# traveller59/spconv

Measured on AMD Instinct MI355X. Metric: active-voxels/sec fwd+bwd, 3x3x3 SubMConv3d C=64, ~100k voxels/scene, higher is better.
Workload: dtype f16; 1 GPU; SubMConv3d 3x3x3 C=64->64 f16, 100000 uniform voxels/scene in 1600x1280x40 (BASELINE configs[1]), 8 distinct scenes per GPU visited round-robin, rulebook reused via indice_key; voxels_per_gpu=100000, launch=hipgraph, steps_per_replay=8, scenes_rotated=8, mask_sort=False, prewarm_steps=0, parallelism=dp1, ranks_seen=1, tree=unknown

## Files before the change

include/spconv_amd.h:

```cpp
#ifndef SPCONV_AMD_H_
#define SPCONV_AMD_H_

#include <stddef.h>
#include <stdint.h>

#ifdef __cplusplus
extern "C" {
#endif

#define SPX_MAX_NDIM 4
#define SPX_UNION_MAX_OPERANDS 8
#define SPX_COLLAPSE_SUM 0
#define SPX_COLLAPSE_MEAN 1
#define SPX_COLLAPSE_MAX 2
#define SPX_SCORE_ABSMEAN 0
#define SPX_SCORE_ABSMAX 1

typedef void *spx_stream_t;

enum spx_dtype { SPX_F32 = 0, SPX_F16 = 1, SPX_BF16 = 2, SPX_I8 = 3, SPX_F64 = 4 };

enum spx_act { SPX_ACT_NONE = 0, SPX_ACT_RELU = 1, SPX_ACT_SIGMOID = 2, SPX_ACT_LEAKY_RELU = 3 };
#define SPX_OUT_CACHED 0x100
#define SPX_TILE_ORDER 0x200

const char *spx_last_error(void);

int spx_version(void);

int spx_set_option(const char *name_h, int value);

long long spx_launch_count(const char *family_h);

int spx_pad_rows(const void *src, void *dst, long long rows, int src_row_bytes, int dst_row_bytes,
                 spx_stream_t stream);

int spx_conv_out_shape(int ndim, const int *in_shape, const int *ksize, const int *stride,
                       const int *padding, const int *dilation, const int *out_padding,
                       int transposed, int *out_shape);


size_t spx_subm_rulebook_ws_bytes(int n, int kv);

int spx_subm_rulebook(const int32_t *indices, int n, int ndim, int batch_size,
                      const int *spatial_shape, const int *ksize, const int *dilation,
                      int32_t *pair_fwd, int32_t *pair_bwd, uint32_t *mask,
                      int32_t *pair_native, int32_t *num_per_loc,
                      void *ws, size_t ws_bytes, spx_stream_t stream);

size_t spx_conv_rulebook_ws_bytes(int n_in, int ndim, const int *ksize, const int *stride,
                                  const int *dilation, int transposed);

int spx_conv_rulebook_count(const int32_t *indices, int n_in, int ndim, int batch_size,
                            const int *in_shape, const int *out_shape, const int *ksize,
                            const int *stride, const int *padding, const int *dilation,
// ... 394 lines not shown
```

spconv_amd/_lib.py:

```python
from __future__ import annotations

import ctypes
import os
import subprocess
from typing import Optional

_HERE = os.path.dirname(os.path.abspath(__file__))
LIB_PATH = os.environ.get("SPX_LIB") or os.path.join(_HERE, "lib", "libspconv_amd.so")

c_int_p = ctypes.POINTER(ctypes.c_int)
c_float_p = ctypes.POINTER(ctypes.c_float)
vp = ctypes.c_void_p

SIGNATURES = {
    "spx_last_error": (ctypes.c_char_p, []),
    "spx_version": (ctypes.c_int, []),
    "spx_set_option": (ctypes.c_int, [ctypes.c_char_p, ctypes.c_int]),
    "spx_conv_out_shape": (ctypes.c_int, [ctypes.c_int] + [c_int_p] * 6 + [ctypes.c_int, c_int_p]),
    "spx_subm_rulebook_ws_bytes": (ctypes.c_size_t, [ctypes.c_int, ctypes.c_int]),
    "spx_subm_rulebook": (ctypes.c_int, [vp, ctypes.c_int, ctypes.c_int, ctypes.c_int, c_int_p,
                                         c_int_p, c_int_p, vp, vp, vp, vp, vp, vp,
                                         ctypes.c_size_t, vp]),
    "spx_conv_rulebook_ws_bytes": (ctypes.c_size_t, [ctypes.c_int, ctypes.c_int, c_int_p, c_int_p,
                                                     c_int_p, ctypes.c_int]),
# ... 84 lines not shown
                                       vp, vp, vp, vp, c_int_p, vp, ctypes.c_size_t, vp]),
    "spx_point2voxel_static_ws_bytes": (ctypes.c_size_t, [ctypes.c_int] * 4 + [c_int_p, ctypes.c_int]),
    "spx_point2voxel_static": (ctypes.c_int, [vp, vp, ctypes.c_int, vp, ctypes.c_int, ctypes.c_int,
                                              ctypes.POINTER(ctypes.c_float), ctypes.POINTER(ctypes.c_float), c_int_p]
                               + [ctypes.c_int] * 5 + [vp] * 6 + [ctypes.c_int, vp, ctypes.c_size_t, vp,
                                                                  ctypes.c_size_t, vp]),
    "spx_hash_ws_bytes": (ctypes.c_size_t, [ctypes.c_int]),
    "spx_hash_clear": (ctypes.c_int, [vp, ctypes.c_int, ctypes.c_int, vp]),
    "spx_hash_insert": (ctypes.c_int, [vp, vp, ctypes.c_int, ctypes.c_int, ctypes.c_int, vp, vp, ctypes.c_int, vp]),
    "spx_hash_query": (ctypes.c_int, [vp, vp, ctypes.c_int, ctypes.c_int, ctypes.c_int, vp, vp, vp, ctypes.c_int, vp]),
    "spx_hash_insert_exist": (ctypes.c_int, [vp, vp, ctypes.c_int, ctypes.c_int, ctypes.c_int, vp, vp, vp,
                                             ctypes.c_int, vp]),
    "spx_hash_assign_arange": (ctypes.c_int, [vp, vp, ctypes.c_int, ctypes.c_int, ctypes.c_int, vp, vp,
                                              ctypes.c_size_t, vp]),
    "spx_hash_items": (ctypes.c_int, [vp, vp, ctypes.c_int, ctypes.c_int, ctypes.c_int, vp, vp, ctypes.c_int, vp,
                                      vp, ctypes.c_size_t, vp]),
    "spx_rankmap_from_sorted": (ctypes.c_int, [vp, ctypes.c_int, ctypes.c_int, ctypes.c_int, c_int_p, vp,
                                               ctypes.c_size_t, vp, vp]),
    "spx_key_argsort_ws_bytes": (ctypes.c_size_t, [ctypes.c_int]),
    "spx_key_argsort": (ctypes.c_int, [vp, ctypes.c_int, ctypes.c_int, ctypes.c_int, c_int_p, vp, vp, vp,
                                       ctypes.c_size_t, vp, vp, vp, ctypes.c_int, vp, ctypes.c_size_t, vp]),
    "spx_pad_rows": (ctypes.c_int, [vp, vp, ctypes.c_longlong, ctypes.c_int, ctypes.c_int, vp]),
    "spx_launch_count": (ctypes.c_longlong, [ctypes.c_char_p]),
    "spx_bias_act_inplace": (ctypes.c_int, [vp, vp, ctypes.c_int, ctypes.c_int, ctypes.c_int,
                                            ctypes.c_int, ctypes.c_float, vp]),
    "spx_dense_ws_bytes": (ctypes.c_size_t, [ctypes.c_int, ctypes.c_int, c_int_p]),
    "spx_dense_map": (ctypes.c_int, [vp, ctypes.c_int, vp, ctypes.c_int, ctypes.c_int, c_int_p, vp, vp]),
    "spx_to_dense": (ctypes.c_int, [vp, ctypes.c_int, ctypes.c_longlong, vp, vp, ctypes.c_int, ctypes.c_int, ctypes.c_int,
                                    ctypes.c_longlong, ctypes.c_int, ctypes.c_int, c_int_p, vp]),
    "spx_dense_gather": (ctypes.c_int, [vp, vp, vp] + [ctypes.c_int] * 6 + [c_int_p, vp]),
    "spx_from_dense_ws_bytes": (ctypes.c_size_t, [ctypes.c_int, ctypes.c_int, c_int_p]),
    "spx_from_dense_count": (ctypes.c_int, [vp] + [ctypes.c_int] * 5 + [c_int_p, vp, ctypes.c_size_t, c_int_p, vp]),
    "spx_from_dense_fill": (ctypes.c_int, [vp] + [ctypes.c_int] * 4 + [c_int_p, vp, ctypes.c_size_t, vp, vp, vp, vp]),
    "spx_union_ws_bytes": (ctypes.c_size_t, [ctypes.c_int, ctypes.c_int, c_int_p, ctypes.c_int, ctypes.c_longlong]),
    "spx_union_count": (ctypes.c_int, [vp, c_int_p, vp, ctypes.c_int, ctypes.c_int, ctypes.c_int, c_int_p, vp,
                                       ctypes.c_size_t, vp, ctypes.c_size_t, c_int_p, vp]),
    "spx_union_fill": (ctypes.c_int, [vp, c_int_p, vp, ctypes.c_int, ctypes.c_int, ctypes.c_int, c_int_p, ctypes.c_int,
                                      ctypes.c_int, vp, vp, vp, vp, ctypes.c_size_t, vp, ctypes.c_size_t, vp]),
    "spx_union_static": (ctypes.c_int, [vp, c_int_p, vp, ctypes.c_int, ctypes.c_int, ctypes.c_int, c_int_p, ctypes.c_int,
                                        vp, vp, vp, vp, vp, ctypes.c_size_t, vp, ctypes.c_size_t, vp]),
    "spx_union_add_fwd": (ctypes.c_int, [vp, c_int_p, ctypes.c_int, vp, ctypes.c_int, ctypes.c_int, ctypes.c_int, vp, vp,
                                         vp]),
    "spx_union_add_bwd": (ctypes.c_int, [vp, ctypes.c_int, vp, vp, c_int_p, ctypes.c_int, ctypes.c_int, ctypes.c_int,
                                         vp]),
    "spx_collapse_ws_bytes": (ctypes.c_size_t, [ctypes.c_int, ctypes.c_int, c_int_p, ctypes.c_int, ctypes.c_longlong]),
    "spx_collapse_count": (ctypes.c_int, [vp, ctypes.c_int, vp, ctypes.c_int, ctypes.c_int, c_int_p, ctypes.c_int, vp,
# ... 134 lines not shown
```

spconv_amd/csrc/counters.cpp:

```cpp
#include "counters.h"

#include <string.h>

#include "../../include/spconv_amd.h"

namespace spx {
std::atomic<long long> g_counters[kCounterSlots];

namespace {
#define SPX_COUNTER_NAME(e, key) key,
const char *const kNames[] = {SPX_COUNTERS(SPX_COUNTER_NAME)};
#undef SPX_COUNTER_NAME
static_assert(sizeof(kNames) / sizeof(kNames[0]) == kNamed, "one name per enumerator");

template <int N>
int index_of(const char *t, const char *const (&names)[N]) {
  for (int i = 0; i < N; ++i)
    if (strcmp(t, names[i]) == 0) return i;
  return -1;
}

int parse_dt(const char *t) {
  static const char *const names[inst::kDts] = {"f16", "bf16", "i8", "f32"};
  return index_of(t, names);
}

int parse_int(const char *t) {
  if (!*t || strlen(t) > 6) return -1;
  int v = 0;
  for (; *t; ++t) {
// ... 66 lines not shown
  if (named >= 0) return named;
  char buf[96];
  if (strlen(key) >= sizeof(buf)) return -1;
  strcpy(buf, key);
  const char *tok[8];
  int n = 0;
  for (char *c = buf, *start = buf;; ++c) {
    if (*c == '/' || *c == 0) {
      if (n == 8) return -1;
      const bool end = *c == 0;
      *c = 0;
      tok[n++] = start;
      start = c + 1;
      if (end) break;
    }
  }
  const int i = instance_slot(tok, n);
  if (i >= 0) return kInstBase + i;
  const int p = pool_key_slot(tok, n);
  return p < 0 ? -1 : kPoolBase + p;
}
}

extern "C" long long spx_launch_count(const char *family_h) {
  const int slot = family_h ? spx::counter_slot(family_h) : -1;
  return slot < 0 ? -1 : spx::g_counters[slot].load(std::memory_order_relaxed);
}
```

spconv_amd/csrc/counters.h:

```cpp
#pragma once
#include <atomic>

namespace spx {

#define SPX_COUNTERS(X)                                                                                               \
  X(kFamV4, "igemm_v4") X(kFamWs, "igemm_ws") X(kFamBwdFused, "igemm_bwd") X(kFamBwdRows, "igemm_bwd_rows")           \
  X(kFamI8Stream, "igemm_i8_stream") X(kFamGeneric, "generic") X(kFamStage2, "wgrad_stage2")                          \
  X(kFamStage2Batch, "wgrad_stage2_batch") X(kFamF64, "igemm_f64") X(kFamV4w, "igemm_v4w")                            \
  X(kHintV4, "sparse_hint/v4") X(kHintBwd, "sparse_hint/bwd")                                                         \
  X(kF64Fwd, "igemm_f64/fwd") X(kF64Dgrad, "igemm_f64/dgrad") X(kF64Wgrad, "wgrad_f64") X(kF64Pool, "pool/f64")       \
  X(kDenseMap, "dense/map") X(kDenseScatterCl, "dense/scatter_cl") X(kDenseScatterCf, "dense/scatter_cf")             \
  X(kDenseGatherCl, "dense/gather_cl") X(kDenseGatherCf, "dense/gather_cf") X(kDenseCompact, "dense/compact")         \
  X(kUnionMark, "union/mark") X(kUnionPrefix, "union/prefix") X(kUnionClaim, "union/claim")                           \
  X(kUnionFill, "union/fill") X(kUnionAddFwd, "union/add_fwd") X(kUnionAddBwd, "union/add_bwd")                       \
  X(kCollapseMark, "collapse/mark") X(kCollapsePrefix, "collapse/prefix") X(kCollapseRank, "collapse/rank")           \
  X(kCollapseList, "collapse/list") X(kCollapseFwd, "collapse/fwd") X(kCollapseBwd, "collapse/bwd")                   \
  X(kPvGroups, "pointvoxel/groups") X(kPvGather, "pointvoxel/gather") X(kPvDecorate, "pointvoxel/decorate")           \
  X(kInterpCornersRanked, "interp/corners_ranked") X(kInterpCornersHash, "interp/corners_hash")                       \
  X(kInterpFwd, "interp/fwd") X(kInterpBwd, "interp/bwd")                                                             \
  X(kQueryRanked, "query/ranked") X(kQueryHash, "query/hash") X(kQueryGroupFwd, "query/group_fwd")                    \
  X(kQueryGroupBwd, "query/group_bwd")                                                                                \
  X(kSampleFps, "sample/fps") X(kSampleBallQuery, "sample/ball_query") X(kSampleKnnQuery, "sample/knn_query")         \
  X(kBoxCorners, "box/corners") X(kBoxPairs, "box/pairs") X(kBoxAligned, "box/aligned") X(kBoxKey, "box/key")         \
  X(kBoxMask, "box/mask") X(kBoxReduce, "box/reduce")                                                                 \
// ... 58 lines not shown
}
constexpr int v4w(int dt, bool bt, int nks, int pk) {
  return kV4w + ((dt * 2 + (bt ? 1 : 0)) * 2 + (nks - 1)) * kWidePks + pk_slot(pk);
}
}

enum PoolDt { kPoolF16 = 0, kPoolBf16, kPoolF32, kPoolF64, kPoolI8, kPoolDts };
constexpr int kPoolOps = 4, kPoolCount = kPoolOps * kPoolDts * 2;
constexpr int pool_slot(int op, int dt, bool scalar) { return (op * kPoolDts + dt) * 2 + (scalar ? 1 : 0); }

constexpr int kInstBase = kNamed, kPoolBase = kInstBase + inst::kCount, kCounterSlots = kPoolBase + kPoolCount;
extern std::atomic<long long> g_counters[kCounterSlots];

inline void count(Counter c) { g_counters[c].fetch_add(1, std::memory_order_relaxed); }
template <int I>
inline void count_inst() {
  static_assert(I >= 0 && I < inst::kCount, "instance counter slot");
  g_counters[kInstBase + I].fetch_add(1, std::memory_order_relaxed);
}
inline void count_pool(int op, int dt, bool scalar) {
  g_counters[kPoolBase + pool_slot(op, dt, scalar)].fetch_add(1, std::memory_order_relaxed);
}

const char *counter_name(int c);
int counter_slot(const char *key);

}
```

spconv_amd/csrc/igemm_bwd.h:

```cpp
#pragma once
#include "igemm_v4.h"

namespace spx {
namespace {

constexpr int kWT = 64;

constexpr int kW2MaxG = 1024;
constexpr int kW2J = 128;
constexpr int kW2Rec = 8;
constexpr int kXcds = 8;


__host__ __device__ inline int plan2_wg(int w) { return 8 + kW2Rec * w; }
__host__ __device__ inline int plan2_kf(int G) { return 8 + kW2Rec * G; }
__host__ __device__ inline int plan2_seg(int G, int kv) { return 8 + kW2Rec * G + kv + 1; }
__host__ __device__ inline int plan2_red(int G, int kv) {
  return (plan2_seg(G, kv) + 3 * (G + kv) + 3) & ~3;
}

__device__ __forceinline__ int wtr_x(int row) { return ((row >> 1) & 1) | (((row >> 3) & 1) << 1); }
__device__ __forceinline__ int wtr_slot(int row, int sl) {
  return row * 128 + ((((sl >> 1) ^ wtr_x(row)) << 5) | ((sl & 1) << 4));
}
// ... 289 lines not shown
int launch_bwd(const GemmParams &p, const Wgrad2Params &q, int n_wgrad_blocks, hipStream_t s) {
  int napp = p.cls ? layout_app_tiles(p.n_dst, 64 * MB) : 0;
  AppShape exact{-1, 0};
  if constexpr (DT == 0 || DT == 1) {
    if (p.cls) exact = app_shape_exact(p.n_dst, 64 * MB, p.app_m, kAppBudget);
  }
  if (exact.napp >= 0) napp = exact.napp;
  const int n_dgrad = div_up(p.n_dst, 64 * MB) + napp;
  GemmRest rr = rest_of(p);
  rr.napp = p.cls ? napp : -1;
  if (exact.napp >= 0) {
    rr.acc_mode = pack_app_shape(p.acc_mode, p.app_m, exact);
    count(kHintBwd);
  }
  constexpr int wgrad_first = 1;
  GemmParams pl = p;
  pl.lpt = p.tile_order && n_dgrad + n_wgrad_blocks > 1024;
  count(kFamBwdFused);
#define SPX_LAUNCH_BWD(NKSV, PKV)                                                                                  \
  do {                                                                                                               \
    count_inst<inst::bwd(COUT, MB, DT, NKSV, PKV)>();                                                                \
    hipLaunchKernelGGL((igemm_bwd_kernel<COUT, MB, DT, NKSV, PKV>), dim3(n_dgrad + n_wgrad_blocks), dim3(kThreads),  \
                       (bwd_smem_bytes<COUT, MB, DT>()), s, p.A, p.B, p.mask, p.argsort, p.pair, p.n_dst,           \
                       p.n_src, p.CIN, p.kv, p.identity_k, v4_flags(pl), rr,                                        \
                       wgrad_first ? ~n_wgrad_blocks : n_dgrad, q);                                                 \
  } while (0)
  const int pk = v4_pack(p, DT, DT == 3 ? 4 : 2, true);
  if constexpr (DT == 0 || DT == 1) {
    if (pk == 32) SPX_LAUNCH_BWD(2, 32);
    else if (pk == 16) SPX_LAUNCH_BWD(2, 16);
    else if (pk == 8) SPX_LAUNCH_BWD(2, 8);
    else if (pk == 4) SPX_LAUNCH_BWD(1, 4);
    else if (pk == 2) SPX_LAUNCH_BWD(1, 2);
    else if (p.CIN * 2 <= 64) SPX_LAUNCH_BWD(1, 1);
    else SPX_LAUNCH_BWD(2, 1);
  } else {
    if (p.CIN * (DT == 3 ? 4 : 2) <= 64) SPX_LAUNCH_BWD(1, 1);
    else SPX_LAUNCH_BWD(2, 1);
  }
#undef SPX_LAUNCH_BWD
  SPX_LAUNCH_CHECK();
  return 0;
}

template <int DT>
int dispatch_bwd(const GemmParams &p, const Wgrad2Params &q, int nwb, hipStream_t s) {
  switch (p.COUT) {
    case 16: return launch_bwd<16, 2, DT>(p, q, nwb, s);
    case 32: return launch_bwd<32, 2, DT>(p, q, nwb, s);
    case 64: return launch_bwd<64, 2, DT>(p, q, nwb, s);
// ... 8 lines not shown
```

spconv_amd/csrc/igemm_defs.h:

```cpp
#pragma once
#include "common.h"

#include <stdlib.h>
#include <type_traits>
#include <utility>

#ifndef SPX_AUX_TABLE
#define SPX_AUX_TABLE 0
#endif
#ifndef SPX_WD
#define SPX_WD 2
#endif
#ifndef SPX_AUX_OUT
#define SPX_AUX_OUT 2
#endif

namespace spx {

struct GemmParams {
  const void *A;
  const void *B;
  void *out;
  const int32_t *pair;
  const uint32_t *mask;
// ... 6 lines not shown
  int tile_order;
  int kbase, mask_words;
  float *acc;
  int acc_mode;
  int act;
  float act_alpha;
  const float *scale;
  const void *add;
  float add_scale;
  int out_dtype;
  int dbg;
  int xcd_rot;
  int lpt;
  const int32_t *cls;
  const uint32_t *mask_rows;
  int app_rows;
  int app_budget;
  int app_m;
  int app_h;
  int dense_hint;
  float *stats;
  const int32_t *n_live;
  int *grid_out;
  int n0;
};

constexpr int kAppBudget = 64;
constexpr int kLayoutMinRows = 32768;
__host__ __device__ inline int layout_mcap(int n) { return ((n / 4 + 63) & ~63) + 256; }
__host__ __device__ inline int layout_app_tiles(int n, int tm) { return (n / 4 + tm - 1) / tm; }

inline void apply_rows_layout(GemmParams &p, int tile_order) {
  p.cls = nullptr;
  p.mask_rows = nullptr;
  p.app_rows = 0;
  p.app_budget = 0;
  p.app_m = -1;
  p.app_h = 0;
  if (tile_order == SPX_ROWS_LAYOUT && p.argsort && p.pair && p.mask) {
    const int32_t *blob = p.argsort;
    const size_t npad = (static_cast<size_t>(p.n_dst) + 63) & ~static_cast<size_t>(63);
    p.cls = blob;
    p.mask_rows = p.mask;
    p.mask = reinterpret_cast<const uint32_t *>(blob + SPX_LAYOUT_HEADER);
    p.argsort = blob + SPX_LAYOUT_HEADER + npad;
    p.tile_order = 0;
// ... 410 lines not shown
```

spconv_amd/csrc/igemm_v4.h:

```cpp
#pragma once
#include "igemm_defs.h"

namespace spx {
namespace {

#ifdef SPX_TIMELINE
constexpr int kTlSlots = 8, kTlMaxWg = 8192;
__device__ unsigned long long g_timeline[kTlMaxWg * kTlSlots];
#define SPX_STAMP(i)                                                                     \
  do {                                                                                   \
    if (threadIdx.x == 0 && blockIdx.x < kTlMaxWg)                                       \
      g_timeline[blockIdx.x * kTlSlots + (i)] = __builtin_amdgcn_s_memtime();            \
  } while (0)
#else
#define SPX_STAMP(i) do {} while (0)
#endif




template <int COUT, int MB, int DT, bool BT, int NKS = 2, int PK = 1, bool WIDE = false>
__device__ __forceinline__ void igemm_v4_body(const GemmParams &p, int block);
__device__ __forceinline__ void unpack_gemm_args(GemmParams &p, const void *argA, const void *argB,
                                                 const uint32_t *arg_mask, const int32_t *arg_argsort,
                                                 const int32_t *arg_pair, int n_dst, int n_src, int CIN,
                                                 int kv, int identity_k, int b_reverse,
                                                 const GemmRest &rest);

template <int COUT, int MB, int DT, bool BT, int NKS = 2, int PK = 1>
__global__ void __launch_bounds__(kThreads)
igemm_v4_kernel(const void *argA, const void *argB, const uint32_t *arg_mask,
                const int32_t *arg_argsort, const int32_t *arg_pair, int n_dst, int n_src, int CIN,
                int kv, int identity_k, int b_reverse, GemmRest rest) {
  GemmParams p;
  unpack_gemm_args(p, argA, argB, arg_mask, arg_argsort, arg_pair, n_dst, n_src, CIN, kv, identity_k,
                   b_reverse, rest);
  igemm_v4_body<COUT, MB, DT, BT, NKS, PK>(p, blockIdx.x);
}

__device__ __forceinline__ void unpack_gemm_args(GemmParams &p, const void *argA, const void *argB,
                                                 const uint32_t *arg_mask, const int32_t *arg_argsort,
                                                 const int32_t *arg_pair, int n_dst, int n_src, int CIN,
                                                 int kv, int identity_k, int b_reverse,
                                                 const GemmRest &rest) {
  p.A = argA;
  p.B = argB;
  p.mask = arg_mask;
  p.argsort = arg_argsort;
  p.pair = arg_pair;
  p.n_dst = n_dst;
  p.n_src = n_src;
  p.CIN = CIN;
  p.kv = kv;
  p.identity_k = identity_k;
  p.b_reverse = b_reverse & 1;
  p.tile_order = (b_reverse >> 1) & 1;
  p.mask_words = ((b_reverse >> 2) & 3) + 1;
  p.kbase = (b_reverse >> 4) & 127;
  p.lpt = (b_reverse >> 11) & 1;
  p.acc = rest.acc;
  p.acc_mode = rest.acc_mode & 3;
  p.out = rest.out;
  p.bias = rest.bias;
  p.strideK = rest.strideK;
  p.strideN = rest.strideN;
  p.strideD = rest.strideD;
  p.COUT = rest.COUT;
  p.act = rest.act;
  p.act_alpha = rest.act_alpha;
  p.scale = rest.scale;
  p.add = rest.add;
  p.add_scale = rest.add_scale;
  p.out_dtype = rest.out_dtype;
  p.dbg = rest.dbg;
  p.xcd_rot = 0;
  p.stats = rest.stats;
  p.n_live = rest.n_live;
  p.app_rows = rest.napp;
  p.app_budget = 0;
  p.app_m = ((rest.acc_mode >> 8) & 0xfffff) - 1;
  p.app_h = ((rest.acc_mode >> 4) & 15) * 16;
  p.cls = nullptr;
// ... 61 lines not shown
        addw[mb][nb] = word;
      } else if (p.out_dtype == SPX_F32) {
        uint32_t d[4];
#pragma unroll
        for (int e = 0; e < 4; ++e) d[e] = __builtin_bit_cast(uint32_t, v[e]);
        store_dwords<4, SPX_AUX_OUT>(d, rO, rowoff[mb] == kOob ? kOob : (rowoff[mb] + nb * 4) * 4u);
      } else {
        uint32_t d[2];
#pragma unroll
        for (int q = 0; q < 2; ++q)
          d[q] = p.out_dtype == SPX_BF16 ? pack2<true>(v[2 * q], v[2 * q + 1])
                                         : pack2<false>(v[2 * q], v[2 * q + 1]);
        store_dwords<2, SPX_AUX_OUT>(d, rO, rowoff[mb] == kOob ? kOob : (rowoff[mb] + nb * 4) * 2u);
      }
    }
  }
  if (p.out_dtype == SPX_I8) {
#pragma unroll
    for (int mb = 0; mb < MB; ++mb) store_dwords<CPL / 4, SPX_AUX_OUT>(addw[mb], rO, rowoff[mb]);
  }

}

template <int COUT, int MB, int DT, bool BT, int NKS, int PK, bool WIDE>
__device__ __forceinline__ void igemm_v4_body(const GemmParams &p, int block) {
  constexpr bool BF16 = DT == 1, I8 = DT == 2, F32 = DT == 3;
  constexpr bool XK = PK >= 8;
  constexpr int PP = XK ? PK / 8 : PK;
  constexpr int T = PP * (XK ? 2 : 1);
  static_assert(PK == 1 || (!I8 && !F32 && (XK ? NKS == 2 : NKS == 1)), "offset packing: 16-bit operands");
  static_assert(PP == 1 || PP == 2 || PP == 4, "offsets per piece");
  constexpr int ES = I8 ? 1 : (F32 ? 4 : 2);
  static_assert(!(I8 && BT), "int8 is forward only");
  constexpr int NB = COUT / 16;
  const int ldo = WIDE ? p.COUT : COUT;
  const int n0 = WIDE ? p.n0 : 0;
  constexpr int TM = 64 * MB;
  constexpr int BROWS = !BT ? (COUT + 31) / 32 : (F32 ? (COUT + 31) / 32 : 2 * ((COUT + 63) / 64));
  constexpr int BA = BROWS < 2 ? 2 : BROWS;
  constexpr int B_BYTES = COUT * kRowBytes;
  constexpr int CPL = NB * 4;
  extern __shared__ __attribute__((aligned(16))) char smem[];
  uint32_t *lds_mask = reinterpret_cast<uint32_t *>(smem + 2 * B_BYTES);
  float *lds_sb = reinterpret_cast<float *>(smem + 2 * B_BYTES + 64);

  SPX_STAMP(0);
  const int tid = threadIdx.x, lane = tid & 63, wave = tid >> 6;
  const int ntiles = (p.n_dst + TM - 1) / TM;
  const int napp = p.cls ? (p.app_rows >= 0 ? p.app_rows : layout_app_tiles(p.n_dst, TM)) : 0;
  const bool app = block < napp;
  int app_m = 0;
  int tile = 0;
  int pos[MB];
  if (app) {
    app_m = p.app_m;
    int h = p.app_h;
    if (app_m < 0) {
      typedef const i32x2 __attribute__((address_space(4))) *cptr_t;
      const i32x2 head = *(cptr_t)(p.cls);
      const int cls = head[0];
      app_m = head[1];
      if (!cls) {
        if constexpr (!I8 && !BT && !WIDE) if (p.stats) wg_bn_stats_empty<COUT>(p.stats, block, static_cast<int>(gridDim.x));
        return;
// ... 11 lines not shown
      const int q = block * h + blk * 16 + (threadIdx.x & 15);
      pos[mb] = (blk * 16 < h && q < app_m) ? q : -1;
    }
    tile = block;
  } else {
    const int bid = block - napp;
    const int rot = (p.xcd_rot + napp) & 7;
    tile = (p.tile_order && p.lpt) ? ntiles - 1 - bid : (rot ? xcd_tile_rot(bid, ntiles, rot) : xcd_tile(bid, ntiles));
#pragma unroll
    for (int mb = 0; mb < MB; ++mb) {
      const int t = tile * TM + ((threadIdx.x >> 6) * MB + mb) * 16 + (threadIdx.x & 15);
      pos[mb] = t < p.n_dst ? t : -1;
    }
  }
  const int mcap = layout_mcap(p.n_dst);
  const int32_t *order_app = p.argsort;
  const uint32_t *maskp = app ? reinterpret_cast<const uint32_t *>(order_app + mcap) : p.mask;
  const int32_t *pairp = app ? order_app + 2 * static_cast<size_t>(mcap) : p.pair;
  const int tbl_rows = app ? mcap : p.n_dst;
  const int lrow = lane & 15, lgrp = lane >> 4;
  const int slot = tid & 7, r0 = tid >> 3;
  constexpr int GL = 4 / PP;
  const int ga = lgrp / GL;
  auto swzB = [](int row, int sl) __attribute__((always_inline)) {
    const int x = ((row >> 1) & 1) | (((row / CPL) & 3) << 1);
    return row * kRowBytes + ((sl ^ x) << 4);
  };
  const uint32_t rowB = static_cast<uint32_t>(p.CIN) * ES;
  const int nchunk = (static_cast<int>(rowB) + kRowBytes - 1) / kRowBytes;
  const bool cfull = (rowB & (kRowBytes - 1)) == 0;

  const uint32_t a_bytes = static_cast<uint32_t>(p.n_src) * rowB;
  const uint32_t w_bytes = static_cast<uint32_t>(p.COUT) * p.kv * rowB;
  const uint32_t pair_bytes = static_cast<uint32_t>(tbl_rows) * 4u;

  const int32_t *olist = (app || !p.cls) ? p.argsort : nullptr;
  const bool by_row = olist && !app && !p.tile_order;
  const __amdgpu_buffer_rsrc_t rO = make_rsrc(olist, olist ? pair_bytes : 0u);
  int glist[MB];
  uint32_t goff[MB];
#pragma unroll
  for (int mb = 0; mb < MB; ++mb) {
    goff[mb] = pos[mb] < 0 ? kOob : static_cast<uint32_t>(pos[mb]) * 4u;
    glist[mb] = static_cast<int>(__builtin_amdgcn_raw_buffer_load_b32(rO, goff[mb], 0, SPX_AUX_TABLE));
  }
  if (by_row) {
#pragma unroll
    for (int mb = 0; mb < MB; ++mb) goff[mb] = pos[mb] < 0 ? kOob : static_cast<uint32_t>(glist[mb]) * 4u;
    asm volatile("" ::: "memory");
  }
// ... 287 lines not shown
    if (!SPX_ABL(p, 1) && !SPX_ABL(p, 2)) store_b(smem + (1 - S) * B_BYTES, WSetN{});
    compute(it0, SET);
    const StepIt it3 = step_next<T>(it2, nchunk);
    if (!SPX_ABL(p, 1) && !SPX_ABL(p, 2)) {
      if constexpr (WD == 2) load_b(it3, WSetN{});
      else load_b(it2, WSetN{});
    }
    __builtin_amdgcn_sched_barrier(0);
    load_idx(it3, std::integral_constant<int, 1 - S>{});
    __builtin_amdgcn_sched_barrier(0);
    load_a(it2, SET);
    it0 = it1;
    it1 = it2;
    it2 = it3;
  };
  SPX_STAMP(3);
  while (it0.k >= 0) {
    step(Set1{});
    step(Set0{});
  }
  SPX_STAMP(4);

  if constexpr (!I8) {
    const bool plain = p.bias == nullptr && p.act == SPX_ACT_NONE;
    const __amdgpu_buffer_rsrc_t rO = make_rsrc(p.out, static_cast<uint32_t>(p.n_dst) * (ldo * ES));
    float bv[CPL];
#pragma unroll
    for (int q = 0; q < CPL; ++q) bv[q] = 0.f;
    if (p.bias) {
#pragma unroll
      for (int q = 0; q < CPL; ++q) {
        if constexpr (F32) bv[q] = static_cast<const float *>(p.bias)[n0 + lgrp * CPL + q];
        else bv[q] = to_float<BF16>(static_cast<const uint16_t *>(p.bias)[n0 + lgrp * CPL + q]);
      }
    }
    if (p.acc_mode) {
      const __amdgpu_buffer_rsrc_t rS = make_rsrc(p.acc, static_cast<uint32_t>(p.n_dst) * (ldo * 4));
#pragma unroll
      for (int mb = 0; mb < MB; ++mb) {
        const uint32_t so = grow[mb] < 0 ? kOob : static_cast<uint32_t>(grow[mb]) * (ldo * 4) + (n0 + lgrp * CPL) * 4;
        uint32_t prev[CPL];
        if (p.acc_mode & 1) load_dwords<CPL>(prev, rS, so);
#pragma unroll
        for (int nb = 0; nb < NB; ++nb)
#pragma unroll
          for (int e = 0; e < 4; ++e) {
            if (p.acc_mode & 1) acc[nb][mb][e] += __builtin_bit_cast(float, prev[nb * 4 + e]);
            prev[nb * 4 + e] = __builtin_bit_cast(uint32_t, static_cast<float>(acc[nb][mb][e]));
          }
        if (p.acc_mode & 2) store_dwords<CPL>(prev, rS, so);
      }
      if (p.acc_mode & 2) return;
    }
#pragma unroll
    for (int mb = 0; mb < MB; ++mb) {
      uint32_t d[F32 ? CPL : CPL / 2];
#pragma unroll
      for (int nb = 0; nb < NB; ++nb) {
#pragma unroll
        for (int h = 0; h < 2; ++h) {
          float v0 = acc[nb][mb][2 * h], v1 = acc[nb][mb][2 * h + 1];
          if (!plain) {
            v0 = apply_act(v0 + bv[nb * 4 + 2 * h], p.act, p.act_alpha);
            v1 = apply_act(v1 + bv[nb * 4 + 2 * h + 1], p.act, p.act_alpha);
          }
          if constexpr (F32) {
            d[nb * 4 + 2 * h] = __builtin_bit_cast(uint32_t, v0);
            d[nb * 4 + 2 * h + 1] = __builtin_bit_cast(uint32_t, v1);
          } else {
            d[nb * 2 + h] = pack2<BF16>(v0, v1);
          }
        }
      }
      const uint32_t vo = grow[mb] < 0 ? kOob
                                       : static_cast<uint32_t>(grow[mb]) * (ldo * ES) + (n0 + lgrp * CPL) * ES;
      if (p.dbg & 0x400) store_dwords<(F32 ? CPL : CPL / 2)>(d, rO, vo);
      else store_dwords<(F32 ? CPL : CPL / 2), 2>(d, rO, vo);
    }
    if constexpr (!BT && !WIDE) {
      if (p.stats) {
        const int st_live = p.n_live ? *p.n_live : 0x7fffffff;
        __syncthreads();
        wg_bn_stats<COUT, CPL, MB, kThreads / 64, (F32 ? 0 : (BF16 ? 2 : 1))>(
            acc, grow, st_live, reinterpret_cast<float *>(smem), p.stats, block, static_cast<int>(gridDim.x));
      }
    }
  } else {
    i8_epilogue<COUT, MB>(p, acc, grow, lgrp, lds_sb, ldo, n0);
  }
  SPX_STAMP(6);
#ifdef SPX_TIMELINE
  asm volatile("s_waitcnt vmcnt(0)" ::: "memory");
  SPX_STAMP(7);
#endif
}

template <int COUT, int MB, int DT = 0>
constexpr size_t v4_smem_bytes() {
  return 2 * static_cast<size_t>(COUT) * kRowBytes + 64 + (DT == 2 ? 2 * static_cast<size_t>(COUT) * 4 : 0);
}

int v4_flags(const GemmParams &p) {
  const int words = p.mask_words > 0 ? p.mask_words : 1;
  return p.b_reverse | (p.tile_order << 1) | ((words - 1) << 2) | (p.kbase << 4) | ((p.lpt ? 1 : 0) << 11) |
         ((p.cls ? 1 : 0) << 12);
}

bool v4_ok(const GemmParams &p, int es = 2, int out_es = 2) {
  const unsigned long long abytes = static_cast<unsigned long long>(p.n_src) * p.CIN * es;
  const unsigned long long pbytes = static_cast<unsigned long long>(p.n_dst) * 4ull;
  const unsigned long long wbytes = static_cast<unsigned long long>(p.COUT) * p.kv * p.CIN * es;
  const unsigned long long obytes = static_cast<unsigned long long>(p.n_dst) * p.COUT * out_es;
  return abytes < 0x7fff0000ull && pbytes < 0x7fff0000ull && wbytes < 0x7fff0000ull &&
         obytes < 0x7fff0000ull;
}

template <int COUT, int MB, int DT>
int launch_v4(const GemmParams &p, hipStream_t s);
GemmRest rest_of(const GemmParams &p);

inline int v4_pack(const GemmParams &p, int DT, int es, bool fused_bwd = false) {
  const int mode = option_int("SPX_PK", 1);
  if ((DT != 0 && DT != 1) || !p.pair || mode == 0) return 1;
  if (static_cast<unsigned long long>(p.n_dst) * 4ull * 32ull >= 0x7fff0000ull) return 1;
  const int rb = p.CIN * es;
  const bool both = mode == 3 || (mode == 1 && fused_bwd);
  if (both) return rb <= 16 ? 32 : (rb <= 32 ? 16 : (rb <= 64 ? 8 : 1));
  return rb <= 16 ? 4 : (rb <= 32 ? 2 : 1);
}

template <int COUT, int MB, int DT>
int launch_v4(const GemmParams &p, hipStream_t s) {
  const int ntiles = div_up(p.n_dst, 64 * MB);
  int napp = p.cls ? (p.app_rows > 0 ? div_up(p.app_rows, 64 * MB) : layout_app_tiles(p.n_dst, 64 * MB)) : 0;
  AppShape exact{-1, 0};
  if constexpr (DT == 0 || DT == 1) {
    if (p.cls && p.app_rows <= 0) exact = app_shape_exact(p.n_dst, 64 * MB, p.app_m, 0);
  }
  if (exact.napp >= 0) napp = exact.napp;
  GemmParams q = p;
  q.lpt = p.tile_order && ntiles > ((DT == 2 || COUT > 64) ? 512 : 1024);
  GemmRest r = rest_of(p);
  r.napp = p.cls ? napp : -1;
  if (exact.napp >= 0) {
    r.acc_mode = pack_app_shape(p.acc_mode, p.app_m, exact);
    count(kHintV4);
  }
  constexpr int es = DT == 2 ? 1 : (DT == 3 ? 4 : 2);
  const bool half = p.CIN * es <= 64;
  const int pk = v4_pack(p, DT, es);
  count(kFamV4);
#define SPX_LAUNCH_V4(BTV, NKSV, PKV)                                                                \
  do {                                                                                                 \
    count_inst<inst::v4(COUT, MB, DT, BTV, NKSV, PKV)>();                                              \
    hipLaunchKernelGGL((igemm_v4_kernel<COUT, MB, DT, BTV, NKSV, PKV>), dim3(napp + ntiles), dim3(kThreads), \
                       (v4_smem_bytes<COUT, MB, DT>()), s, p.A, p.B, p.mask, p.argsort, p.pair, p.n_dst,  \
                       p.n_src, p.CIN, p.kv, p.identity_k, v4_flags(q), r);                            \
  } while (0)
  if (p.grid_out) *p.grid_out = (p.stats && DT != 2 && p.strideD == 1 && !p.acc_mode) ? napp + ntiles : 0;
  if (DT == 2 || p.strideD == 1) {
    if constexpr (DT == 0 || DT == 1) {
      if (pk == 32) SPX_LAUNCH_V4(false, 2, 32);
      else if (pk == 16) SPX_LAUNCH_V4(false, 2, 16);
      else if (pk == 8) SPX_LAUNCH_V4(false, 2, 8);
      else if (pk == 4) SPX_LAUNCH_V4(false, 1, 4);
      else if (pk == 2) SPX_LAUNCH_V4(false, 1, 2);
      else if (half) SPX_LAUNCH_V4(false, 1, 1);
      else SPX_LAUNCH_V4(false, 2, 1);
    } else {
      if (half) SPX_LAUNCH_V4(false, 1, 1);
      else SPX_LAUNCH_V4(false, 2, 1);
    }
  } else if constexpr (DT != 2) {
    if constexpr (DT == 0 || DT == 1) {
      if (pk == 32) SPX_LAUNCH_V4(true, 2, 32);
      else if (pk == 16) SPX_LAUNCH_V4(true, 2, 16);
      else if (pk == 8) SPX_LAUNCH_V4(true, 2, 8);
      else if (pk == 4) SPX_LAUNCH_V4(true, 1, 4);
      else if (pk == 2) SPX_LAUNCH_V4(true, 1, 2);
      else if (half) SPX_LAUNCH_V4(true, 1, 1);
// ... 201 lines not shown
```

Before: 4.172 billion voxels/s.

## Add lean single-offset main-tile path for C=64 f16 implicit GEMM

Adds a specialized 'lean' path for the main (non-appendix) tiles of the v4 implicit-GEMM kernel when operands are 16-bit with 64 in/out channels and the appendix layout is exact. Those tiles then handle only the identity kernel offset: one weight slice loaded into LDS, direct row loads of A, two MFMA k-steps and a shared epilogue, skipping the general gather and mask loop. The epilogue is factored into a reusable function. The change also raises launch-bounds occupancy hints for that instantiation, which may add register pressure, and adds a launch counter for the lean path.

```diff
diff --git a/include/spconv_amd.h b/include/spconv_amd.h
--- a/include/spconv_amd.h
+++ b/include/spconv_amd.h
@@ -31,6 +31,7 @@
 int spx_set_option(const char *name_h, int value);
 
 long long spx_launch_count(const char *family_h);
+long long spx_lean_main_launches(void);
 
 int spx_pad_rows(const void *src, void *dst, long long rows, int src_row_bytes, int dst_row_bytes,
                  spx_stream_t stream);
diff --git a/spconv_amd/_lib.py b/spconv_amd/_lib.py
--- a/spconv_amd/_lib.py
+++ b/spconv_amd/_lib.py
@@ -130,6 +130,7 @@
                                        ctypes.c_size_t, vp, vp, vp, ctypes.c_int, vp, ctypes.c_size_t, vp]),
     "spx_pad_rows": (ctypes.c_int, [vp, vp, ctypes.c_longlong, ctypes.c_int, ctypes.c_int, vp]),
     "spx_launch_count": (ctypes.c_longlong, [ctypes.c_char_p]),
+    "spx_lean_main_launches": (ctypes.c_longlong, []),
     "spx_bias_act_inplace": (ctypes.c_int, [vp, vp, ctypes.c_int, ctypes.c_int, ctypes.c_int,
                                             ctypes.c_int, ctypes.c_float, vp]),
     "spx_dense_ws_bytes": (ctypes.c_size_t, [ctypes.c_int, ctypes.c_int, c_int_p]),
diff --git a/spconv_amd/csrc/counters.cpp b/spconv_amd/csrc/counters.cpp
--- a/spconv_amd/csrc/counters.cpp
+++ b/spconv_amd/csrc/counters.cpp
@@ -6,6 +6,7 @@
 
 namespace spx {
 std::atomic<long long> g_counters[kCounterSlots];
+std::atomic<long long> g_lean_main_launches{0};
 
 namespace {
 #define SPX_COUNTER_NAME(e, key) key,
@@ -118,6 +119,10 @@
 }
 }
 
+extern "C" long long spx_lean_main_launches(void) {
+  return spx::g_lean_main_launches.load(std::memory_order_relaxed);
+}
+
 extern "C" long long spx_launch_count(const char *family_h) {
   const int slot = family_h ? spx::counter_slot(family_h) : -1;
   return slot < 0 ? -1 : spx::g_counters[slot].load(std::memory_order_relaxed);
diff --git a/spconv_amd/csrc/counters.h b/spconv_amd/csrc/counters.h
--- a/spconv_amd/csrc/counters.h
+++ b/spconv_amd/csrc/counters.h
@@ -104,6 +104,9 @@
   g_counters[kPoolBase + pool_slot(op, dt, scalar)].fetch_add(1, std::memory_order_relaxed);
 }
 
+extern std::atomic<long long> g_lean_main_launches;
+inline void count_lean_main() { g_lean_main_launches.fetch_add(1, std::memory_order_relaxed); }
+
 const char *counter_name(int c);
 int counter_slot(const char *key);
 
diff --git a/spconv_amd/csrc/igemm_bwd.h b/spconv_amd/csrc/igemm_bwd.h
--- a/spconv_amd/csrc/igemm_bwd.h
+++ b/spconv_amd/csrc/igemm_bwd.h
@@ -335,10 +335,12 @@
     count_inst<inst::bwd(COUT, MB, DT, NKSV, PKV)>();                                                                \
     hipLaunchKernelGGL((igemm_bwd_kernel<COUT, MB, DT, NKSV, PKV>), dim3(n_dgrad + n_wgrad_blocks), dim3(kThreads),  \
                        (bwd_smem_bytes<COUT, MB, DT>()), s, p.A, p.B, p.mask, p.argsort, p.pair, p.n_dst,           \
-                       p.n_src, p.CIN, p.kv, p.identity_k, v4_flags(pl), rr,                                        \
+                       p.n_src, p.CIN, p.kv, p.identity_k, v4_flags(pl) | lean, rr,                                 \
                        wgrad_first ? ~n_wgrad_blocks : n_dgrad, q);                                                 \
   } while (0)
   const int pk = v4_pack(p, DT, DT == 3 ? 4 : 2, true);
+  const int lean = (exact.napp >= 0 && v4_lean_ok<COUT, DT>(p, p.CIN * 2 <= 64 ? 1 : 2, pk)) ? 1 << 13 : 0;
+  if (lean) count_lean_main();
   if constexpr (DT == 0 || DT == 1) {
     if (pk == 32) SPX_LAUNCH_BWD(2, 32);
     else if (pk == 16) SPX_LAUNCH_BWD(2, 16);
diff --git a/spconv_amd/csrc/igemm_defs.h b/spconv_amd/csrc/igemm_defs.h
--- a/spconv_amd/csrc/igemm_defs.h
+++ b/spconv_amd/csrc/igemm_defs.h
@@ -52,6 +52,7 @@
   float *stats;
   const int32_t *n_live;
   int *grid_out;
+  int lean;
   int n0;
 };
 
diff --git a/spconv_amd/csrc/igemm_v4.h b/spconv_amd/csrc/igemm_v4.h
--- a/spconv_amd/csrc/igemm_v4.h
+++ b/spconv_amd/csrc/igemm_v4.h
@@ -28,7 +28,7 @@
                                                  const GemmRest &rest);
 
 template <int COUT, int MB, int DT, bool BT, int NKS = 2, int PK = 1>
-__global__ void __launch_bounds__(kThreads)
+__global__ void __launch_bounds__(kThreads, ((DT == 0 || DT == 1) && COUT == 64 && NKS == 2 && PK == 1) ? 4 : 1)
 igemm_v4_kernel(const void *argA, const void *argB, const uint32_t *arg_mask,
                 const int32_t *arg_argsort, const int32_t *arg_pair, int n_dst, int n_src, int CIN,
                 int kv, int identity_k, int b_reverse, GemmRest rest) {
@@ -58,6 +58,7 @@
   p.mask_words = ((b_reverse >> 2) & 3) + 1;
   p.kbase = (b_reverse >> 4) & 127;
   p.lpt = (b_reverse >> 11) & 1;
+  p.lean = (b_reverse >> 13) & 1;
   p.acc = rest.acc;
   p.acc_mode = rest.acc_mode & 3;
   p.out = rest.out;
@@ -165,9 +166,176 @@
 
 }
 
+template <int CPL>
+__device__ __forceinline__ int v4_swz_b(int row, int sl) {
+  const int x = ((row >> 1) & 1) | (((row / CPL) & 3) << 1);
+  return row * kRowBytes + ((sl ^ x) << 4);
+}
+
+template <int COUT, int MB, int DT, bool BT, bool WIDE, typename Acc>
+__device__ __forceinline__ bool v4_epilogue(const GemmParams &p, Acc (&acc)[COUT / 16][MB], const int (&grow)[MB], int lgrp,
+                                            int ldo, int n0, int block) {
+  constexpr bool BF16 = DT == 1, F32 = DT == 3;
+  constexpr int NB = COUT / 16, CPL = NB * 4, ES = F32 ? 4 : 2;
+  extern __shared__ __attribute__((aligned(16))) char smem[];
+  const bool plain = p.bias == nullptr && p.act == SPX_ACT_NONE;
+  const __amdgpu_buffer_rsrc_t rO = make_rsrc(p.out, static_cast<uint32_t>(p.n_dst) * (ldo * ES));
+  float bv[CPL];
+#pragma unroll
+  for (int q = 0; q < CPL; ++q) bv[q] = 0.f;
+  if (p.bias) {
+#pragma unroll
+    for (int q = 0; q < CPL; ++q) {
+      if constexpr (F32) bv[q] = static_cast<const float *>(p.bias)[n0 + lgrp * CPL + q];
+      else bv[q] = to_float<BF16>(static_cast<const uint16_t *>(p.bias)[n0 + lgrp * CPL + q]);
+    }
+  }
+  if (p.acc_mode) {
+    const __amdgpu_buffer_rsrc_t rS = make_rsrc(p.acc, static_cast<uint32_t>(p.n_dst) * (ldo * 4));
+#pragma unroll
+    for (int mb = 0; mb < MB; ++mb) {
+      const uint32_t so = grow[mb] < 0 ? kOob : static_cast<uint32_t>(grow[mb]) * (ldo * 4) + (n0 + lgrp * CPL) * 4;
+      uint32_t prev[CPL];
+      if (p.acc_mode & 1) load_dwords<CPL>(prev, rS, so);
+#pragma unroll
+      for (int nb = 0; nb < NB; ++nb)
+#pragma unroll
+        for (int e = 0; e < 4; ++e) {
+          if (p.acc_mode & 1) acc[nb][mb][e] += __builtin_bit_cast(float, prev[nb * 4 + e]);
+          prev[nb * 4 + e] = __builtin_bit_cast(uint32_t, static_cast<float>(acc[nb][mb][e]));
+        }
+      if (p.acc_mode & 2) store_dwords<CPL>(prev, rS, so);
+    }
+    if (p.acc_mode & 2) return true;
+  }
+#pragma unroll
+  for (int mb = 0; mb < MB; ++mb) {
+    uint32_t d[F32 ? CPL : CPL / 2];
+#pragma unroll
+    for (int nb = 0; nb < NB; ++nb) {
+#pragma unroll
+      for (int h = 0; h < 2; ++h) {
+        float v0 = acc[nb][mb][2 * h], v1 = acc[nb][mb][2 * h + 1];
+        if (!plain) {
+          v0 = apply_act(v0 + bv[nb * 4 + 2 * h], p.act, p.act_alpha);
+          v1 = apply_act(v1 + bv[nb * 4 + 2 * h + 1], p.act, p.act_alpha);
+        }
+        if constexpr (F32) {
+          d[nb * 4 + 2 * h] = __builtin_bit_cast(uint32_t, v0);
+          d[nb * 4 + 2 * h + 1] = __builtin_bit_cast(uint32_t, v1);
+        } else {
+          d[nb * 2 + h] = pack2<BF16>(v0, v1);
+        }
+      }
+    }
+    const uint32_t vo = grow[mb] < 0 ? kOob
+                                     : static_cast<uint32_t>(grow[mb]) * (ldo * ES) + (n0 + lgrp * CPL) * ES;
+    if (p.dbg & 0x400) store_dwords<(F32 ? CPL : CPL / 2)>(d, rO, vo);
+    else store_dwords<(F32 ? CPL : CPL / 2), 2>(d, rO, vo);
+  }
+  if constexpr (!BT && !WIDE) {
+    if (p.stats) {
+      const int st_live = p.n_live ? *p.n_live : 0x7fffffff;
+      __syncthreads();
+      wg_bn_stats<COUT, CPL, MB, kThreads / 64, (F32 ? 0 : (BF16 ? 2 : 1))>(
+          acc, grow, st_live, reinterpret_cast<float *>(smem), p.stats, block, static_cast<int>(gridDim.x));
+    }
+  }
+  return false;
+}
+
+template <int COUT, int MB, int DT, bool BT>
+__device__ __forceinline__ void v4_lean_main(const GemmParams &p, int block, int napp) {
+  constexpr int NB = COUT / 16, CPL = NB * 4, TM = 64 * MB;
+  static_assert((DT == 0 || DT == 1) && COUT == 64, "one-step main tiles: 16-bit operands, 64 output channels");
+  extern __shared__ __attribute__((aligned(16))) char smem[];
+  SPX_STAMP(0);
+  const int tid = threadIdx.x, lane = tid & 63, wave = tid >> 6;
+  const int lrow = lane & 15, lgrp = lane >> 4;
+  const int ntiles = (p.n_dst + TM - 1) / TM;
+  const int bid = block - napp;
+  const int rot = (p.xcd_rot + napp) & 7;
+  const int tile = rot ? xcd_tile_rot(bid, ntiles, rot) : xcd_tile(bid, ntiles);
+  int grow[MB];
+  uint32_t mraw[MB];
+  u32x4 areg[MB][2];
+  const __amdgpu_buffer_rsrc_t rM = make_rsrc(p.mask, static_cast<uint32_t>(p.n_dst) * 4u);
+  const __amdgpu_buffer_rsrc_t rA = make_rsrc(p.A, static_cast<uint32_t>(p.n_src) * kRowBytes);
+#pragma unroll
+  for (int mb = 0; mb < MB; ++mb) {
+    const int t = tile * TM + (wave * MB + mb) * 16 + lrow;
+    grow[mb] = t < p.n_dst ? t : -1;
+    mraw[mb] = __builtin_amdgcn_raw_buffer_load_b32(rM, grow[mb] < 0 ? kOob : static_cast<uint32_t>(t) * 4u, 0, SPX_AUX_TABLE);
+  }
+  const int kb = p.b_reverse ? p.kv - 1 - p.identity_k : p.identity_k;
+  const uint32_t so = static_cast<uint32_t>(kb) * static_cast<uint32_t>(p.strideK) * 2u;
+  const __amdgpu_buffer_rsrc_t rW =
+      make_rsrc(p.B, static_cast<uint32_t>(p.COUT) * p.kv * static_cast<uint32_t>(kRowBytes));
+  const int slot = tid & 7, r0 = tid >> 3;
+  u32x4 breg[2];
+#pragma unroll
+  for (int j = 0; j < 2; ++j) {
+    const uint32_t o = !BT ? static_cast<uint32_t>(r0 + 32 * j) * static_cast<uint32_t>(p.strideN) * 2u + slot * 16u
+                           : (static_cast<uint32_t>(2 * r0 + j) * static_cast<uint32_t>(p.strideD) + slot * 8u) * 2u;
+    breg[j] = __builtin_amdgcn_raw_buffer_load_b128(rW, o, so, 0);
+  }
+#pragma unroll
+  for (int mb = 0; mb < MB; ++mb)
+#pragma unroll
+    for (int ks = 0; ks < 2; ++ks)
+      areg[mb][ks] = __builtin_amdgcn_raw_buffer_load_b128(
+          rA, grow[mb] < 0 ? kOob : static_cast<uint32_t>(grow[mb]) * kRowBytes + (ks * 64 + lgrp * 16), 0, 0);
+  __builtin_amdgcn_sched_barrier(0);
+  SPX_STAMP(1);
+  if constexpr (!BT) {
+#pragma unroll
+    for (int j = 0; j < 2; ++j) *reinterpret_cast<u32x4 *>(smem + v4_swz_b<CPL>(r0 + 32 * j, slot)) = breg[j];
+  } else {
+#pragma unroll
+    for (int e = 0; e < 8; ++e) {
+      const int n = slot * 8 + e;
+      const uint32_t ev = breg[0][e >> 1], od = breg[1][e >> 1];
+      const uint32_t v = (e & 1) ? __builtin_amdgcn_perm(od, ev, 0x07060302u) : __builtin_amdgcn_perm(od, ev, 0x05040100u);
+      *reinterpret_cast<uint32_t *>(smem + v4_swz_b<CPL>(n, r0 >> 2) + (r0 & 3) * 4) = v;
+    }
+  }
+  __syncthreads();
+  SPX_STAMP(2);
+  u32x4 fb[2][NB];
+#pragma unroll
+  for (int ks = 0; ks < 2; ++ks)
+#pragma unroll
+    for (int nb = 0; nb < NB; ++nb)
+      fb[ks][nb] = *reinterpret_cast<const u32x4 *>(
+          smem + v4_swz_b<CPL>((lrow >> 2) * CPL + nb * 4 + (lrow & 3), ks * 4 + lgrp));
+  SPX_STAMP(3);
+  f32x4 acc[NB][MB];
+#pragma unroll
+  for (int nb = 0; nb < NB; ++nb)
+#pragma unroll
+    for (int mb = 0; mb < MB; ++mb) acc[nb][mb] = f32x4{0.f, 0.f, 0.f, 0.f};
+#pragma unroll
+  for (int ks = 0; ks < 2; ++ks)
+#pragma unroll
+    for (int nb = 0; nb < NB; ++nb)
+#pragma unroll
+      for (int mb = 0; mb < MB; ++mb)
+        acc[nb][mb] = mfma_step<DT>(__builtin_bit_cast(uint4, fb[ks][nb]), __builtin_bit_cast(uint4, areg[mb][ks]), acc[nb][mb]);
+  SPX_STAMP(4);
+#pragma unroll
+  for (int mb = 0; mb < MB; ++mb)
+    if (mraw[mb] == 0u) grow[mb] = -1;
+  v4_epilogue<COUT, MB, DT, BT, false>(p, acc, grow, lgrp, COUT, 0, block);
+  SPX_STAMP(6);
+#ifdef SPX_TIMELINE
+  asm volatile("s_waitcnt vmcnt(0)" ::: "memory");
+  SPX_STAMP(7);
+#endif
+}
+
 template <int COUT, int MB, int DT, bool BT, int NKS, int PK, bool WIDE>
 __device__ __forceinline__ void igemm_v4_body(const GemmParams &p, int block) {
-  constexpr bool BF16 = DT == 1, I8 = DT == 2, F32 = DT == 3;
+  constexpr bool I8 = DT == 2, F32 = DT == 3;
   constexpr bool XK = PK >= 8;
   constexpr int PP = XK ? PK / 8 : PK;
   constexpr int T = PP * (XK ? 2 : 1);
@@ -183,6 +351,12 @@
   constexpr int BA = BROWS < 2 ? 2 : BROWS;
   constexpr int B_BYTES = COUT * kRowBytes;
   constexpr int CPL = NB * 4;
+  if constexpr ((DT == 0 || DT == 1) && COUT == 64 && NKS == 2 && PK == 1 && !WIDE) {
+    if (p.lean && block >= p.app_rows) {
+      v4_lean_main<COUT, MB, DT, BT>(p, block, p.app_rows);
+      return;
+    }
+  }
   extern __shared__ __attribute__((aligned(16))) char smem[];
   uint32_t *lds_mask = reinterpret_cast<uint32_t *>(smem + 2 * B_BYTES);
   float *lds_sb = reinterpret_cast<float *>(smem + 2 * B_BYTES + 64);
@@ -240,10 +414,7 @@
   const int slot = tid & 7, r0 = tid >> 3;
   constexpr int GL = 4 / PP;
   const int ga = lgrp / GL;
-  auto swzB = [](int row, int sl) __attribute__((always_inline)) {
-    const int x = ((row >> 1) & 1) | (((row / CPL) & 3) << 1);
-    return row * kRowBytes + ((sl ^ x) << 4);
-  };
+  auto swzB = [](int row, int sl) __attribute__((always_inline)) { return v4_swz_b<CPL>(row, sl); };
   const uint32_t rowB = static_cast<uint32_t>(p.CIN) * ES;
   const int nchunk = (static_cast<int>(rowB) + kRowBytes - 1) / kRowBytes;
   const bool cfull = (rowB & (kRowBytes - 1)) == 0;
@@ -577,69 +748,7 @@
   SPX_STAMP(4);
 
   if constexpr (!I8) {
-    const bool plain = p.bias == nullptr && p.act == SPX_ACT_NONE;
-    const __amdgpu_buffer_rsrc_t rO = make_rsrc(p.out, static_cast<uint32_t>(p.n_dst) * (ldo * ES));
-    float bv[CPL];
-#pragma unroll
-    for (int q = 0; q < CPL; ++q) bv[q] = 0.f;
-    if (p.bias) {
-#pragma unroll
-      for (int q = 0; q < CPL; ++q) {
-        if constexpr (F32) bv[q] = static_cast<const float *>(p.bias)[n0 + lgrp * CPL + q];
-        else bv[q] = to_float<BF16>(static_cast<const uint16_t *>(p.bias)[n0 + lgrp * CPL + q]);
-      }
-    }
-    if (p.acc_mode) {
-      const __amdgpu_buffer_rsrc_t rS = make_rsrc(p.acc, static_cast<uint32_t>(p.n_dst) * (ldo * 4));
-#pragma unroll
-      for (int mb = 0; mb < MB; ++mb) {
-        const uint32_t so = grow[mb] < 0 ? kOob : static_cast<uint32_t>(grow[mb]) * (ldo * 4) + (n0 + lgrp * CPL) * 4;
-        uint32_t prev[CPL];
-        if (p.acc_mode & 1) load_dwords<CPL>(prev, rS, so);
-#pragma unroll
-        for (int nb = 0; nb < NB; ++nb)
-#pragma unroll
-          for (int e = 0; e < 4; ++e) {
-            if (p.acc_mode & 1) acc[nb][mb][e] += __builtin_bit_cast(float, prev[nb * 4 + e]);
-            prev[nb * 4 + e] = __builtin_bit_cast(uint32_t, static_cast<float>(acc[nb][mb][e]));
-          }
-        if (p.acc_mode & 2) store_dwords<CPL>(prev, rS, so);
-      }
-      if (p.acc_mode & 2) return;
-    }
-#pragma unroll
-    for (int mb = 0; mb < MB; ++mb) {
-      uint32_t d[F32 ? CPL : CPL / 2];
-#pragma unroll
-      for (int nb = 0; nb < NB; ++nb) {
-#pragma unroll
-        for (int h = 0; h < 2; ++h) {
-          float v0 = acc[nb][mb][2 * h], v1 = acc[nb][mb][2 * h + 1];
-          if (!plain) {
-            v0 = apply_act(v0 + bv[nb * 4 + 2 * h], p.act, p.act_alpha);
-            v1 = apply_act(v1 + bv[nb * 4 + 2 * h + 1], p.act, p.act_alpha);
-          }
-          if constexpr (F32) {
-            d[nb * 4 + 2 * h] = __builtin_bit_cast(uint32_t, v0);
-            d[nb * 4 + 2 * h + 1] = __builtin_bit_cast(uint32_t, v1);
-          } else {
-            d[nb * 2 + h] = pack2<BF16>(v0, v1);
-          }
-        }
-      }
-      const uint32_t vo = grow[mb] < 0 ? kOob
-                                       : static_cast<uint32_t>(grow[mb]) * (ldo * ES) + (n0 + lgrp * CPL) * ES;
-      if (p.dbg & 0x400) store_dwords<(F32 ? CPL : CPL / 2)>(d, rO, vo);
-      else store_dwords<(F32 ? CPL : CPL / 2), 2>(d, rO, vo);
-    }
-    if constexpr (!BT && !WIDE) {
-      if (p.stats) {
-        const int st_live = p.n_live ? *p.n_live : 0x7fffffff;
-        __syncthreads();
-        wg_bn_stats<COUT, CPL, MB, kThreads / 64, (F32 ? 0 : (BF16 ? 2 : 1))>(
-            acc, grow, st_live, reinterpret_cast<float *>(smem), p.stats, block, static_cast<int>(gridDim.x));
-      }
-    }
+    if (v4_epilogue<COUT, MB, DT, BT, WIDE>(p, acc, grow, lgrp, ldo, n0, block)) return;
   } else {
     i8_epilogue<COUT, MB>(p, acc, grow, lgrp, lds_sb, ldo, n0);
   }
@@ -659,6 +768,15 @@
   const int words = p.mask_words > 0 ? p.mask_words : 1;
   return p.b_reverse | (p.tile_order << 1) | ((words - 1) << 2) | (p.kbase << 4) | ((p.lpt ? 1 : 0) << 11) |
          ((p.cls ? 1 : 0) << 12);
+}
+
+template <int COUT, int DT>
+bool v4_lean_ok(const GemmParams &p, int nks, int pk) {
+  if constexpr ((DT == 0 || DT == 1) && COUT == 64) {
+    return nks == 2 && pk == 1 && p.cls && p.app_m >= 0 && p.CIN == 64 && p.COUT == 64 && p.identity_k >= 0 &&
+           p.identity_k < p.kv && !(p.acc_mode & 3) && p.kbase == 0 && p.mask_words <= 1 && !p.tile_order;
+  }
+  return false;
 }
 
 bool v4_ok(const GemmParams &p, int es = 2, int out_es = 2) {
@@ -704,13 +822,15 @@
   constexpr int es = DT == 2 ? 1 : (DT == 3 ? 4 : 2);
   const bool half = p.CIN * es <= 64;
   const int pk = v4_pack(p, DT, es);
+  const int lean = (exact.napp >= 0 && v4_lean_ok<COUT, DT>(p, half ? 1 : 2, pk)) ? 1 << 13 : 0;
+  if (lean) count_lean_main();
   count(kFamV4);
 #define SPX_LAUNCH_V4(BTV, NKSV, PKV)                                                                \
   do {                                                                                                 \
     count_inst<inst::v4(COUT, MB, DT, BTV, NKSV, PKV)>();                                              \
     hipLaunchKernelGGL((igemm_v4_kernel<COUT, MB, DT, BTV, NKSV, PKV>), dim3(napp + ntiles), dim3(kThreads), \
                        (v4_smem_bytes<COUT, MB, DT>()), s, p.A, p.B, p.mask, p.argsort, p.pair, p.n_dst,  \
-                       p.n_src, p.CIN, p.kv, p.identity_k, v4_flags(q), r);                            \
+                       p.n_src, p.CIN, p.kv, p.identity_k, v4_flags(q) | lean, r);                     \
   } while (0)
   if (p.grid_out) *p.grid_out = (p.stats && DT != 2 && p.strideD == 1 && !p.acc_mode) ? napp + ntiles : 0;
   if (DT == 2 || p.strideD == 1) {
```

New measurement: 4.270 billion voxels/s (median of 6 runs). +2.3%, better.
